# burn-research/OpenMEASURE

Measured on AMD Instinct MI355X. Metric: SPR fit+reconstruct throughput (GB/s snapshot matrix), higher is better.
Workload: dtype f64

## Files before the change

openmeasure_amd/csrc/common.hpp:

```cpp
#pragma once
#include <hip/hip_runtime.h>
#include <stdint.h>
#include <stdio.h>

#include "spr_hip.h"

typedef double f64x4 __attribute__((ext_vector_type(4)));
typedef double f64x2 __attribute__((ext_vector_type(2)));

void spr_set_error(const char *fmt, ...);

#define SPR_REQUIRE(cond, code, ...)      \
  do {                                    \
    if (!(cond)) {                        \
      spr_set_error(__VA_ARGS__);         \
      return (code);                      \
    }                                     \
  } while (0)

#define SPR_HIP_TRY(expr)                                                          \
  do {                                                                             \
    hipError_t e__ = (expr);                                                       \
    if (e__ != hipSuccess) {                                                       \
      spr_set_error("%s failed: %s (%s:%d)", #expr, hipGetErrorString(e__),       \
                    __FILE__, __LINE__);                                           \
      return SPR_E_HIP;                                                            \
    }                                                                              \
  } while (0)

#define SPR_LAUNCH_CHECK()                                                         \
  do {                                                                             \
    hipError_t e__ = hipGetLastError();                                            \
    if (e__ != hipSuccess) {                                                       \
      spr_set_error("kernel launch failed: %s (%s:%d)", hipGetErrorString(e__),   \
                    __FILE__, __LINE__);                                           \
      return SPR_E_HIP;                                                            \
    }                                                                              \
  } while (0)

int spr_cached_cus();

struct SegPlan {
  int64_t row0, n_rows, n_points;
  int32_t n_features;
  int32_t total_wg;
  int32_t chunk_rows;
};

__host__ __device__ inline void seg_range(const SegPlan &p, int f, int64_t &lo, int64_t &hi) {
  int64_t glo = (int64_t)f * p.n_points, ghi = glo + p.n_points;
  if (glo < p.row0) glo = p.row0;
  if (ghi > p.row0 + p.n_rows) ghi = p.row0 + p.n_rows;
  if (ghi < glo) ghi = glo;
  lo = glo - p.row0;
  hi = ghi - p.row0;
}

__host__ __device__ inline int seg_wgs(const SegPlan &p, int64_t rows) {
  if (rows <= 0) return 0;
  int64_t w = rows * (int64_t)p.total_wg / p.n_rows;
  int64_t chunks = (rows + p.chunk_rows - 1) / p.chunk_rows;
  if (w > chunks) w = chunks;
  if (w < 1) w = 1;
  return (int)w;
}

__host__ __device__ inline int seg_first_feature(const SegPlan &p) { return (int)(p.row0 / p.n_points); }
__host__ __device__ inline int seg_last_feature(const SegPlan &p) {
  int64_t f = (p.row0 + p.n_rows - 1) / p.n_points;
  if (f > p.n_features - 1) f = p.n_features - 1;
  return (int)f;
}

// ... 65 lines not shown
```

openmeasure_amd/csrc/project_ws.hip:

```cpp
#include <type_traits>

#include "rowtile.hpp"

namespace {

#ifndef WS_ABLATE
#define WS_ABLATE 0
#endif
constexpr int WS_WAVES = 8;
constexpr int WS_ROWS = 16 * WS_WAVES;

template <int RT> struct WsLds { static constexpr int NC = 16 * RT, LDW = NC; static_assert(RT % 2 == 0, "column tiles come in pairs"); };

template <typename TX> struct WsPiece;
template <> struct WsPiece<double> { f64x2 a, b; };
template <> struct WsPiece<float> { float x, y, z, w; };

template <int VEC, typename TX>
__device__ inline WsPiece<TX> ws_load(const TX *__restrict__ rp, int col0, int m) {
  WsPiece<TX> p;
  if constexpr (std::is_same<TX, double>::value) {
    if (VEC) {
      p.a = *reinterpret_cast<const f64x2 *>(rp + col0);
      p.b = *reinterpret_cast<const f64x2 *>(rp + col0 + 2);
    } else {
      p.a.x = rp[col0 < m ? col0 : 0];         p.a.y = rp[col0 + 1 < m ? col0 + 1 : 0];
      p.b.x = rp[col0 + 2 < m ? col0 + 2 : 0]; p.b.y = rp[col0 + 3 < m ? col0 + 3 : 0];
    }
  } else {
    if (VEC) {
      const float4 v = *reinterpret_cast<const float4 *>(rp + col0);
      p.x = v.x; p.y = v.y; p.z = v.z; p.w = v.w;
    } else {
      p.x = rp[col0 < m ? col0 : 0];         p.y = rp[col0 + 1 < m ? col0 + 1 : 0];
      p.z = rp[col0 + 2 < m ? col0 + 2 : 0]; p.w = rp[col0 + 3 < m ? col0 + 3 : 0];
    }
  }
  return p;
}

template <typename TX>
__device__ inline double ws_elem(const WsPiece<TX> &p, int t) {
  if constexpr (std::is_same<TX, double>::value) return t == 0 ? p.a.x : t == 1 ? p.a.y : t == 2 ? p.b.x : p.b.y;
  else return (double)(t == 0 ? p.x : t == 1 ? p.y : t == 2 ? p.z : p.w);
}

template <int MT, int RT, int VEC, typename TX, typename TU, bool NRM>
__global__ __launch_bounds__(WS_WAVES * 64) void project_ws_kernel(
    const TX *__restrict__ X, int64_t ldx, int m, int center_i, SegPlan plan, const double *__restrict__ inv_scale,
    const double *__restrict__ rowmean, const double *__restrict__ W, int r, TU *__restrict__ Ur, int64_t ldu,
    double *__restrict__ nrm2) {
  constexpr int K = 16 * MT, NJ = MT;
  constexpr int NC = WsLds<RT>::NC, LDW = WsLds<RT>::LDW;
  __shared__ double Wl[K * LDW];

  int f, wl, wpf, base;
  int64_t lo, hi;
  if (!seg_locate(plan, blockIdx.x, f, wl, wpf, base, lo, hi)) return;

  const int lane = threadIdx.x & 63;
  const int wave = __builtin_amdgcn_readfirstlane(threadIdx.x >> 6);
  const int li = lane & 15, kk = lane >> 4;
  const double isc = inv_scale[f];

  for (int e = threadIdx.x; e < K * NC; e += WS_WAVES * 64) {
    const int k = e / NC, c = e - k * NC;
    Wl[k * LDW + (c >> 5) * 32 + (c & 15) * 2 + ((c >> 4) & 1)] = (k < m && c < r) ? W[(int64_t)k * r + c] * isc : 0.0;
  }
  __syncthreads();
  double wbar[RT];
#pragma unroll
  for (int ct = 0; ct < RT; ++ct) {
    double sacc = 0.0;
    if (center_i != 0) {
      for (int k = kk; k < K; k += 4) sacc += Wl[k * LDW + (ct >> 1) * 32 + li * 2 + (ct & 1)];
      sacc += __shfl_xor(sacc, 16, 64);
      sacc += __shfl_xor(sacc, 32, 64);
    }
    wbar[ct] = sacc;
  }

  const int64_t nchunks = (hi - lo + WS_ROWS - 1) / WS_ROWS;
  int64_t c = wl;
  if (c >= nchunks) return;
  const double *wb = Wl + (4 * kk) * LDW + 2 * li;
  const double *wb_hi = wb + 128 * LDW;

  auto row_ptr = [&](int64_t cc) {
    int64_t row = lo + cc * WS_ROWS + 16 * wave + li;
    row = row < hi ? row : hi - 1;
    return X + row * ldx;
  };
  WsPiece<TX> areg[NJ];
  {
    const TX *rp = row_ptr(c);
#pragma unroll
    for (int j = 0; j < NJ; ++j) areg[j] = ws_load<VEC, TX>(rp, 16 * j + 4 * kk, m);
  }
  while (c < nchunks) {
    const int64_t cn = c + wpf;
    const TX *rpn = row_ptr(cn < nchunks ? cn : c);
    const int64_t blk0 = lo + c * WS_ROWS + 16 * wave;
    double mu[4];
#pragma unroll
    for (int i = 0; i < 4; ++i) {
      const int64_t rr = blk0 + kk + 4 * i;
      const double v = rowmean[rr < hi ? rr : hi - 1];
      mu[i] = center_i != 0 ? v : 0.0;
    }
    f64x4 acc[RT];
#pragma unroll
    for (int ct = 0; ct < RT; ++ct) acc[ct] = (f64x4){0.0, 0.0, 0.0, 0.0};
    f64x2 bcur[RT / 2], bnxt[RT / 2];
#pragma unroll
    for (int p = 0; p < RT / 2; ++p) bcur[p] = *reinterpret_cast<const f64x2 *>(wb + 32 * p);
#pragma unroll
    for (int j = 0; j < NJ; ++j) {
// ... 22 lines not shown
        for (int p = 0; p < RT / 2; ++p) bcur[p] = bnxt[p];
      }
    }
    {
      const bool full = (blk0 + 16 <= hi) && (r == NC);
      TU *up = Ur + (blk0 + kk) * ldu + li;
      double q[4] = {0.0, 0.0, 0.0, 0.0};
#pragma unroll
      for (int ct = 0; ct < RT; ++ct) {
        const double s[4] = {acc[ct].x - mu[0] * wbar[ct], acc[ct].y - mu[1] * wbar[ct],
                             acc[ct].z - mu[2] * wbar[ct], acc[ct].w - mu[3] * wbar[ct]};
        if (NRM) {
#pragma unroll
          for (int i = 0; i < 4; ++i) { const double v = (double)(TU)s[i]; q[i] = fma(v, v, q[i]); }
        }
        if (full) {
#pragma unroll
          for (int i = 0; i < 4; ++i) up[4 * i * ldu + 16 * ct] = (TU)s[i];
        } else if (16 * ct + li < r) {
#pragma unroll
          for (int i = 0; i < 4; ++i)
            if (blk0 + kk + 4 * i < hi) up[4 * i * ldu + 16 * ct] = (TU)s[i];
        }
      }
      if (NRM) {
#pragma unroll
        for (int i = 0; i < 4; ++i) {
          const double t = group_sum_t<16>(q[i]);
          if (li == i && blk0 + kk + 4 * i < hi) nrm2[blk0 + kk + 4 * i] = t;
        }
      }
    }
    c = cn;
  }
}

template <int MT, int RT, typename TX, typename TU>
int ws_launch(const TX *X, int64_t n_rows, int32_t m, int64_t ldx, int64_t row0, int64_t n_points, int32_t n_features,
              int center, const double *inv_scale, const double *rowmean, const double *W, int32_t r, TU *Ur,
              int64_t ldu, int accumulate, double *nrm2, hipStream_t st) {
  const int cus = spr_cached_cus();
  SegPlan plan;
  plan.row0 = row0; plan.n_rows = n_rows; plan.n_points = n_points; plan.n_features = n_features;
  static const int narrow_per_cu = [] { const char *e = getenv("SPR_WS_WG_PER_CU"); const int v = e ? atoi(e) : 2; return v >= 1 && v <= 4 ? v : 2; }();
  plan.total_wg = (cus > 0 ? cus : 256) * (MT <= 4 ? narrow_per_cu : 1);
  plan.chunk_rows = WS_ROWS;
  const int grid = seg_total_wgs(plan);
  const bool vec = (m == 16 * MT) && ((sizeof(TX) * ldx) % 16 == 0) && ((reinterpret_cast<uintptr_t>(X) & 15) == 0);
  if (!vec) return SPR_E_UNSUPPORTED;
  if (nrm2)
    hipLaunchKernelGGL((project_ws_kernel<MT, RT, 1, TX, TU, true>), dim3(grid), dim3(WS_WAVES * 64), 0, st, X, ldx, (int)m,
                       center, plan, inv_scale, rowmean, W, (int)r, Ur, ldu, nrm2);
  else
    hipLaunchKernelGGL((project_ws_kernel<MT, RT, 1, TX, TU, false>), dim3(grid), dim3(WS_WAVES * 64), 0, st, X, ldx, (int)m,
                       center, plan, inv_scale, rowmean, W, (int)r, Ur, ldu, nrm2);
  SPR_LAUNCH_CHECK();
  return SPR_OK;
}

}

#include "project_ws.hpp"

template <typename TX, typename TU>
int spr_project_ws(const TX *d_X, int64_t n_rows, int32_t m, int64_t ldx, int64_t row0, int64_t n_points,
                   int32_t n_features, int32_t center, const double *d_inv_scale, const double *d_rowmean,
                   const double *d_W, int32_t r, TU *d_Ur, int64_t ldu, int32_t accumulate, double *d_rownorm2,
                   hipStream_t st) {
  if (accumulate) return SPR_E_UNSUPPORTED;
  const int mt = spr_round_mt(m);
  const int need = (r + 15) / 16;
  const int rt = need <= 2 ? 2 : need <= 4 ? 4 : 0;
#define WS(MTV, RTV)                                                                                             \
  if (mt == MTV && rt == RTV)                                                                                    \
    return ws_launch<MTV, RTV, TX, TU>(d_X, n_rows, m, ldx, row0, n_points, n_features, center, d_inv_scale,   \
                                        d_rowmean, d_W, r, d_Ur, ldu, accumulate, d_rownorm2, st)
#ifdef PROJ_WS_LAB
  WS(16, 4);
#else
  WS(4, 2); WS(4, 4); WS(8, 2); WS(8, 4); WS(12, 2); WS(12, 4); WS(16, 2); WS(16, 4);
#endif
#undef WS
  return SPR_E_UNSUPPORTED;
}

template int spr_project_ws<double, double>(const double *, int64_t, int32_t, int64_t, int64_t, int64_t, int32_t, int32_t,
                                            const double *, const double *, const double *, int32_t, double *, int64_t,
                                            int32_t, double *, hipStream_t);
// ... 9 lines not shown
```

openmeasure_amd/csrc/runtime.hip:

```cpp
#include <stdarg.h>
#include <stdlib.h>
#include <string.h>

#include "common.hpp"

namespace {
thread_local char g_err[512] = "";
}

void spr_set_error(const char *fmt, ...) {
  va_list ap;
  va_start(ap, fmt);
  vsnprintf(g_err, sizeof(g_err), fmt, ap);
  va_end(ap);
}

int spr_cached_cus() {
  static int cus = 0;
  if (cus) return cus;
  int dev = 0;
  hipDeviceProp_t prop;
  if (hipGetDevice(&dev) != hipSuccess || hipGetDeviceProperties(&prop, dev) != hipSuccess) return 0;
  cus = prop.multiProcessorCount;
  if (const char *e = getenv("SPR_RESERVE_CUS")) {
    const int k = atoi(e);
    if (k > 0 && k < cus) cus -= k;
  }
  return cus;
}

extern "C" int spr_abi_version(void) { return SPR_ABI_VERSION; }

extern "C" const char *spr_last_error(void) { return g_err; }

extern "C" int spr_device_cus(int *out_cus) {
  SPR_REQUIRE(out_cus != nullptr, SPR_E_INVALID, "spr_device_cus: NULL output");
  const int c = spr_cached_cus();
  SPR_REQUIRE(c > 0, SPR_E_HIP, "spr_device_cus: no HIP device");
  *out_cus = c;
  return SPR_OK;
}

namespace {
__global__ __launch_bounds__(256) void upload_kernel(const uint64_t *__restrict__ src, uint64_t *__restrict__ dst,
                                                     int64_t n_words) {
  for (int64_t i = (int64_t)blockIdx.x * 256 + threadIdx.x; i < n_words; i += (int64_t)gridDim.x * 256)
    dst[i] = __builtin_nontemporal_load(src + i);
// ... 42 lines not shown
```

openmeasure_amd/csrc/stats_gram.hip:

```cpp
#include <stdlib.h>

#include <type_traits>

#include "rowtile.hpp"

#ifndef GRAM_UNIT_PAIRING
#define GRAM_UNIT_PAIRING 1
#endif
#ifndef GRAM_ABLATE
#define GRAM_ABLATE 0
#endif
#if GRAM_ABLATE == 1
#define GRAM_MFMA(a, b, c) ({ asm volatile("" ::"v"(a), "v"(b)); (c); })
#else
#define GRAM_MFMA(a, b, c) __builtin_amdgcn_mfma_f64_16x16x4f64((a), (b), (c), 0, 0, 0)
#endif

namespace {

template <int MT>
struct GramShape {
  static constexpr int MPAD = 16 * MT;
  static constexpr int MP = MPAD + ((MT % 2 == 0) ? 16 : 0);
  static constexpr int T = MT * (MT + 1) / 2;
  static constexpr int NU = (MT + 1) / 2;
};

template <int MT> struct GramCfg;
template <> struct GramCfg<1>  { static constexpr int NW = 8,  R = 64, KS = 8; static constexpr bool DBUF = true; static constexpr int LPRMAX = 16; };
template <> struct GramCfg<2>  { static constexpr int NW = 8,  R = 32, KS = 8; static constexpr bool DBUF = true; static constexpr int LPRMAX = 16; };
template <> struct GramCfg<3>  { static constexpr int NW = 8,  R = 64, KS = 4; static constexpr bool DBUF = true; static constexpr int LPRMAX = 16; };
#ifndef GRAM4_R
#define GRAM4_R 64
#define GRAM4_LPR 8
#endif
template <> struct GramCfg<4>  { static constexpr int NW = 8,  R = GRAM4_R, KS = 4; static constexpr bool DBUF = true; static constexpr int LPRMAX = GRAM4_LPR; };
// ... 146 lines not shown
    }
  }
  if (KSO == KS || ks == 0) {
    double *sp = slab + ((int64_t)blockIdx.x * KSO + (KSO == KS ? ks : 0)) * T * 256 + lane;
#pragma unroll
    for (int j = 0; j < NA; ++j) {
      double *tp = sp + (int64_t)tri_index(MT, RA, RA + j) * 256;
      tp[0] = accA[j].x; tp[64] = accA[j].y; tp[128] = accA[j].z; tp[192] = accA[j].w;
    }
#pragma unroll
    for (int j = 0; j < NB; ++j) {
      double *tp = sp + (int64_t)tri_index(MT, RB, RB + j) * 256;
      tp[0] = accB[j].x; tp[64] = accB[j].y; tp[128] = accB[j].z; tp[192] = accB[j].w;
    }
  }
  if ((lane % RT::LPR) == 0) {
    double *q = stat_part + ((int64_t)blockIdx.x * RT::ROWS_PER_IT + wave * RT::RPW + lane / RT::LPR) * 3;
    q[0] = st.cnt; q[1] = st.mean(); q[2] = st.m2();
  }
}

__device__ inline void chan_merge(double &n, double &mu, double &m2, double nb, double mb, double sb) {
  if (nb > 0.0) {
    const double tot = n + nb, d = mb - mu;
    mu += d * nb / tot;
    m2 += sb + d * d * n * nb / tot;
    n = tot;
  }
}

template <int MT, int U, typename TX, bool EXT, bool SUMS>
__device__ inline void gram_wave_own(const TX *__restrict__ X, int64_t ldx, int64_t lo, int64_t hi, int wl, int wpf, int ks,
                                     int wave, int lane, double *__restrict__ lds0, double *__restrict__ lds1,
                                     double *__restrict__ rowmean, double *__restrict__ slab, double *__restrict__ rowsum) {
  using S = GramShape<MT>;
  using C = GramCfg<MT>;
  constexpr int R = C::R, KS = C::KS, NW = C::NW, MP = S::MP, T = S::T;
  constexpr int KROWS = R / KS, KSTEPS = KROWS / 4;
  constexpr int RA = U, RB = MT - 1 - U;
  constexpr int NA = MT - RA;
  constexpr int NB = (RB != RA) ? MT - RB : 0;
  using RT = RowTile<MT, R, MP, NW, C::LPRMAX, TX>;

  f64x4 accA[NA];
  f64x4 accB[NB > 0 ? NB : 1];
#pragma unroll
  for (int j = 0; j < NA; ++j) accA[j] = (f64x4){0.0, 0.0, 0.0, 0.0};
#pragma unroll
  for (int j = 0; j < NB; ++j) accB[j] = (f64x4){0.0, 0.0, 0.0, 0.0};

  RT tile;
  const int64_t nchunks = (hi - lo + R - 1) / R;
  const int64_t lane_off = (int64_t)(wave * RT::RPW + lane / RT::LPR) * ldx;
  auto base_of = [&](int64_t row0) { return X + row0 * ldx; };
  int64_t c = wl;
  int64_t crow0 = lo + c * R;
#pragma unroll
  for (int it = 0; it < RT::IT; ++it) tile.template load_pass_own<EXT>(it, base_of(crow0), ldx, lane_off, hi - crow0, wave, lane, rowmean, crow0);
  if (crow0 + R <= hi) {
#pragma unroll
    for (int it = 0; it < RT::IT; ++it) tile.template center_store_own<true, EXT, SUMS>(it, lds0, crow0, hi - crow0, wave, lane, rowmean, rowsum);
  } else {
#pragma unroll
    for (int it = 0; it < RT::IT; ++it) tile.template center_store_own<false, EXT, SUMS>(it, lds0, crow0, hi - crow0, wave, lane, rowmean, rowsum);
  }
  int64_t cn = c + wpf;
  int64_t nrow0 = (cn < nchunks) ? lo + cn * R : hi;
// ... 23 lines not shown
      double op[2][NA];
#pragma unroll
      for (int j = 0; j < NA; ++j) op[0][j] = p[16 * j];
#pragma unroll
      for (int k = 0; k < KSTEPS; ++k) {
        if (k + 1 < KSTEPS) {
#pragma unroll
          for (int j = 0; j < NA; ++j) op[(k + 1) & 1][j] = p[(k + 1) * 4 * MP + 16 * j];
        }
#pragma unroll
        for (int j = 0; j < NA; ++j) accA[j] = GRAM_MFMA(op[k & 1][0], op[k & 1][j], accA[j]);
#pragma unroll
        for (int j = 0; j < NB; ++j) accB[j] = GRAM_MFMA(op[k & 1][RB - RA], op[k & 1][RB - RA + j], accB[j]);
        if (nfull) stage(std::true_type{}, k); else stage(std::false_type{}, k);
      }
    } else {
#pragma unroll
      for (int k = 0; k < KSTEPS; ++k) {
        double op[NA];
#pragma unroll
        for (int j = 0; j < NA; ++j) op[j] = p[k * 4 * MP + 16 * j];
#pragma unroll
        for (int j = 0; j < NA; ++j) accA[j] = GRAM_MFMA(op[0], op[j], accA[j]);
#pragma unroll
        for (int j = 0; j < NB; ++j) accB[j] = GRAM_MFMA(op[RB - RA], op[RB - RA + j], accB[j]);
        if (nfull) stage(std::true_type{}, k); else stage(std::false_type{}, k);
      }
    }
    buf ^= 1;
    c = cn;
    cn = c2;
    nrow0 = n2row0;
  }
  double *sp = slab + ((int64_t)blockIdx.x * KS + ks) * T * 256 + lane;
#pragma unroll
  for (int j = 0; j < NA; ++j) {
    double *tp = sp + (int64_t)tri_index(MT, RA, RA + j) * 256;
    tp[0] = accA[j].x; tp[64] = accA[j].y; tp[128] = accA[j].z; tp[192] = accA[j].w;
  }
#pragma unroll
  for (int j = 0; j < NB; ++j) {
    double *tp = sp + (int64_t)tri_index(MT, RB, RB + j) * 256;
    tp[0] = accB[j].x; tp[64] = accB[j].y; tp[128] = accB[j].z; tp[192] = accB[j].w;
  }
}

template <int MT, typename TX, bool EXT, bool SUMS>
__global__ __launch_bounds__(GramCfg<MT>::NW * 64) void stats_gram_own_kernel(
    const TX *__restrict__ X, int64_t ldx, SegPlan plan, double *__restrict__ rowmean, double *__restrict__ slab,
    double *__restrict__ rowsum) {
  using S = GramShape<MT>;
  using C = GramCfg<MT>;
  constexpr int NU = S::NU;
  __shared__ double lds[2][C::R * S::MP];
  int f, wl, wpf, base;
  int64_t lo, hi;
  if (!seg_locate(plan, blockIdx.x, f, wl, wpf, base, lo, hi)) return;
  const int lane = threadIdx.x & 63;
  const int wave = __builtin_amdgcn_readfirstlane(threadIdx.x >> 6);
  const int ks = wave / NU;
  const int unit = (GRAM_UNIT_PAIRING && NU == 8 && C::KS == 1) ? ((wave < 4) ? wave : 11 - wave) : wave % NU;
#define GRAM_UNIT(UV)                                                                                          \
  case UV:                                                                                                     \
    if constexpr (UV < NU)                                                                                     \
      gram_wave_own<MT, UV, TX, EXT, SUMS>(X, ldx, lo, hi, wl, wpf, ks, wave, lane, lds[0], lds[1], rowmean, slab, rowsum); \
    break;
  switch (unit) {
    GRAM_UNIT(0) GRAM_UNIT(1) GRAM_UNIT(2) GRAM_UNIT(3) GRAM_UNIT(4) GRAM_UNIT(5) GRAM_UNIT(6) GRAM_UNIT(7)
    default: break;
  }
#undef GRAM_UNIT
}

constexpr int RS_THREADS = 1024;
__global__ __launch_bounds__(RS_THREADS) void gram_rowmean_stats_kernel(const double *__restrict__ rowmean, SegPlan plan,
                                                                        int slots_per_wg, double *__restrict__ stat_part) {
  __shared__ double sn[RS_THREADS / 64], smu[RS_THREADS / 64], sm2[RS_THREADS / 64];
  int f, wl, wpf, base;
  int64_t lo, hi;
  if (!seg_locate(plan, blockIdx.x, f, wl, wpf, base, lo, hi)) return;
  const int lane = threadIdx.x & 63, wave = threadIdx.x >> 6;
  RowStats st;
  st.init();
  const int64_t step = (int64_t)wpf * RS_THREADS;
  int64_t row = lo + (int64_t)wl * RS_THREADS + threadIdx.x;
  for (; row + 3 * step < hi; row += 4 * step) {
    const double a = rowmean[row], b = rowmean[row + step], c = rowmean[row + 2 * step], d = rowmean[row + 3 * step];
    st.push(a, true); st.push(b, true); st.push(c, true); st.push(d, true);
  }
  for (; row < hi; row += step) st.push(rowmean[row], true);
  double n = st.cnt, mu = st.mean(), m2 = st.m2();
  for (int o = 32; o > 0; o >>= 1) {
    const double on = __shfl_down(n, o, 64), om = __shfl_down(mu, o, 64), os = __shfl_down(m2, o, 64);
    chan_merge(n, mu, m2, on, om, os);
  }
  if (lane == 0) { sn[wave] = n; smu[wave] = mu; sm2[wave] = m2; }
  __syncthreads();
  double *q = stat_part + (int64_t)blockIdx.x * slots_per_wg * 3;
  if (threadIdx.x == 0) {
    n = 0.0; mu = 0.0; m2 = 0.0;
    for (int w = 0; w < RS_THREADS / 64; ++w) chan_merge(n, mu, m2, sn[w], smu[w], sm2[w]);
    q[0] = n; q[1] = mu; q[2] = m2;
  }
  for (int e = 3 + threadIdx.x; e < slots_per_wg * 3; e += RS_THREADS) q[e] = 0.0;
}

template <int MT, int VEC, typename TX>
__global__ __launch_bounds__(GramCfg<MT>::NW * 64) void stats_gram_kernel(
    const TX *__restrict__ X, int64_t ldx, int m, int center_i, SegPlan plan,
    double *__restrict__ rowmean, double *__restrict__ stat_part, double *__restrict__ slab, double *__restrict__ rowsum) {
  using S = GramShape<MT>;
  using C = GramCfg<MT>;
  constexpr int NU = S::NU;
  static_assert(NU * C::KS == C::NW, "waves = units x k slices");
  __shared__ double lds[2][C::R * S::MP];

  int f, wl, wpf, base;
  int64_t lo, hi;
  if (!seg_locate(plan, blockIdx.x, f, wl, wpf, base, lo, hi)) return;

  const int lane = threadIdx.x & 63;
  const int wave = __builtin_amdgcn_readfirstlane(threadIdx.x >> 6);
  const int unit = wave % NU, ks = wave / NU;
#define GRAM_UNIT(UV)                                                                                        \
  case UV:                                                                                                   \
    if constexpr (UV < NU)                                                                                   \
      gram_wave<MT, UV, VEC, TX>(X, ldx, m, center_i, lo, hi, wl, wpf, ks, wave, lane, lds[0],    \
                        lds[1], rowmean, stat_part, slab, rowsum);                                           \
    break;
  switch (unit) {
    GRAM_UNIT(0) GRAM_UNIT(1) GRAM_UNIT(2) GRAM_UNIT(3) GRAM_UNIT(4) GRAM_UNIT(5) GRAM_UNIT(6) GRAM_UNIT(7)
    default: break;
  }
#undef GRAM_UNIT
}

template <int MT>
__global__ __launch_bounds__(1024) void gram_finalize_kernel(
    const double *__restrict__ slab, const double *__restrict__ stat_part, int m, SegPlan plan,
    int slots_per_wg, double *__restrict__ gram, double *__restrict__ fstats, int ldg, int origin) {
  constexpr int T = GramShape<MT>::T;
  constexpr int KS = GramOut<MT>::KSO;
  __shared__ double red[4][256];
  const int f = blockIdx.y;
  const int tile = blockIdx.x;
  int base = 0, wpf = 0;
  {
    int acc = 0;
    const int f0 = seg_first_feature(plan), f1 = seg_last_feature(plan);
    for (int ff = f0; ff <= f1; ++ff) {
      int64_t lo, hi;
      seg_range(plan, ff, lo, hi);
      const int w = seg_wgs(plan, hi - lo);
      if (ff == f) { base = acc; wpf = w; }
      acc += w;
    }
  }
  int ti, tj;
  tile_coords<MT>(tile, ti, tj);
  const int e = threadIdx.x & 255, g = threadIdx.x >> 8;
  const int np = wpf * KS;
  const double *sp = slab + ((int64_t)base * KS * T + tile) * 256 + e;
  const int64_t stride = (int64_t)T * 256;
  double s0 = 0.0, s1 = 0.0, s2 = 0.0, s3 = 0.0;
  int p = g;
  for (; p + 12 < np; p += 16) {
    s0 += sp[p * stride];
    s1 += sp[(p + 4) * stride];
    s2 += sp[(p + 8) * stride];
    s3 += sp[(p + 12) * stride];
  }
  for (; p < np; p += 4) s0 += sp[p * stride];
  red[g][e] = (s0 + s1) + (s2 + s3);
  __syncthreads();
  if (g == 0) {
    const double sum = (red[0][e] + red[1][e]) + (red[2][e] + red[3][e]);
    const int l = e & 63, reg = e >> 6;
    const int gi = ti * 16 + (l >> 4) + 4 * reg, gj = tj * 16 + (l & 15);
    if (gi < m && gj < m) {
      double *G = gram + (int64_t)f * ldg * ldg + (int64_t)origin * ldg + origin;
// ... 22 lines not shown
    }
  }
}

template <int MT>
int occupancy_wgs() {
  static int cached = 0;
  if (cached) return cached;
  int per_cu = 0;
  if (hipOccupancyMaxActiveBlocksPerMultiprocessor(&per_cu, stats_gram_kernel<MT, 2, double>, GramCfg<MT>::NW * 64, 0) != hipSuccess ||
      per_cu < 1)
    per_cu = 1;
  if (per_cu > 4) per_cu = 4;
  const int cus = spr_cached_cus();
  cached = per_cu * (cus > 0 ? cus : 256);
  return cached;
}

template <int MT>
SegPlan make_plan(int64_t n_rows, int64_t row0, int64_t n_points, int32_t n_features) {
  SegPlan p;
  p.row0 = row0; p.n_rows = n_rows; p.n_points = n_points; p.n_features = n_features;
  p.total_wg = occupancy_wgs<MT>();
  p.chunk_rows = GramCfg<MT>::R;
  return p;
}

template <int MT>
size_t workspace_bytes(int32_t n_features) {
  using RT = RowTile<MT, GramCfg<MT>::R, GramShape<MT>::MP, GramCfg<MT>::NW, GramCfg<MT>::LPRMAX>;
  const int64_t max_grid = (int64_t)occupancy_wgs<MT>() + n_features;
  return (size_t)max_grid * GramCfg<MT>::KS * GramShape<MT>::T * 256 * sizeof(double) +
         (size_t)max_grid * RT::ROWS_PER_IT * 3 * sizeof(double);
}

template <int MT, typename TX>
int launch(const TX *X, int64_t n_rows, int32_t m, int64_t ldx, int64_t row0, int64_t n_points,
           int32_t n_features, int center, double *rowmean, void *ws, size_t ws_bytes, hipStream_t st,
           double *rowsum = nullptr) {
  SPR_REQUIRE(ws_bytes >= workspace_bytes<MT>(n_features), SPR_E_WORKSPACE,
              "spr_stats_gram_f64: workspace %zu < %zu", ws_bytes, workspace_bytes<MT>(n_features));
  SPR_REQUIRE(!rowsum || center == 2, SPR_E_INVALID, "spr_stats_gram: row sums are an output of centre mode 2 only");
  SegPlan plan = make_plan<MT>(n_rows, row0, n_points, n_features);
  const int grid = seg_total_wgs(plan);
  const int64_t max_grid = (int64_t)occupancy_wgs<MT>() + n_features;
  SPR_REQUIRE(grid >= 1 && grid <= max_grid, SPR_E_INVALID, "spr_stats_gram_f64: bad grid %d", grid);
  double *slab = static_cast<double *>(ws);
  double *stat_part = slab + (size_t)max_grid * GramCfg<MT>::KS * GramShape<MT>::T * 256;
  const int vec_ok = (m % 2 == 0) && (ldx % 2 == 0) && ((reinterpret_cast<uintptr_t>(X) & (2 * sizeof(TX) - 1)) == 0);
  const int lm = vec_ok ? ((m == 16 * MT) ? 2 : 1) : 0;
#define SG_LAUNCH(LM)                                                                                         \
  hipLaunchKernelGGL((stats_gram_kernel<MT, LM, TX>), dim3(grid), dim3(GramCfg<MT>::NW * 64), 0, st, X, ldx, (int)m, \
                     center, plan, rowmean, stat_part, slab, rowsum)
  using RTL = RowTile<MT, GramCfg<MT>::R, GramShape<MT>::MP, GramCfg<MT>::NW, GramCfg<MT>::LPRMAX, TX>;
  static const bool own_on = [] { const char *e = getenv("SPR_GRAM_OWN"); return !(e && e[0] == '0'); }();
  if (MT >= 8 && lm == 2 && (center == 1 || center == 2) && own_on && (sizeof(TX) * ldx) % 16 == 0 &&
      (reinterpret_cast<uintptr_t>(X) & 15) == 0) {
    if constexpr (MT >= 8) {
      if (center == 1)
        hipLaunchKernelGGL((stats_gram_own_kernel<MT, TX, false, false>), dim3(grid), dim3(GramCfg<MT>::NW * 64), 0, st, X, ldx,
                           plan, rowmean, slab, rowsum);
      else if (!rowsum)
        hipLaunchKernelGGL((stats_gram_own_kernel<MT, TX, true, false>), dim3(grid), dim3(GramCfg<MT>::NW * 64), 0, st, X, ldx,
                           plan, rowmean, slab, rowsum);
      else
        hipLaunchKernelGGL((stats_gram_own_kernel<MT, TX, true, true>), dim3(grid), dim3(GramCfg<MT>::NW * 64), 0, st, X, ldx,
                           plan, rowmean, slab, rowsum);
      SPR_LAUNCH_CHECK();
      hipLaunchKernelGGL(gram_rowmean_stats_kernel, dim3(grid), dim3(RS_THREADS), 0, st, rowmean, plan, (int)RTL::ROWS_PER_IT,
                         stat_part);
      SPR_LAUNCH_CHECK();
      return SPR_OK;
    }
  }
  if (lm == 2) SG_LAUNCH(2);
  else if (lm == 1) SG_LAUNCH(1);
  else SG_LAUNCH(0);
#undef SG_LAUNCH
  SPR_LAUNCH_CHECK();
  return SPR_OK;
}

template <int MT>
int launch_finalize(int64_t n_rows, int32_t m, int64_t row0, int64_t n_points, int32_t n_features,
                    double *fstats, double *gram, int ldg, int origin, const void *ws, size_t ws_bytes,
                    hipStream_t st) {
  using RT = RowTile<MT, GramCfg<MT>::R, GramShape<MT>::MP, GramCfg<MT>::NW, GramCfg<MT>::LPRMAX>;
  SPR_REQUIRE(ws_bytes >= workspace_bytes<MT>(n_features), SPR_E_WORKSPACE,
              "spr_stats_gram_finalize_f64: workspace %zu < %zu", ws_bytes, workspace_bytes<MT>(n_features));
  SegPlan plan = make_plan<MT>(n_rows, row0, n_points, n_features);
  const int64_t max_grid = (int64_t)occupancy_wgs<MT>() + n_features;
  const double *slab = static_cast<const double *>(ws);
  const double *stat_part = slab + (size_t)max_grid * GramCfg<MT>::KS * GramShape<MT>::T * 256;
  hipLaunchKernelGGL(gram_finalize_kernel<MT>, dim3(GramShape<MT>::T, n_features), dim3(1024), 0, st, slab,
                     stat_part, (int)m, plan, (int)RT::ROWS_PER_IT, gram, fstats, ldg, origin);
  SPR_LAUNCH_CHECK();
  return SPR_OK;
}

int check_args(const char *who, const void *X, int64_t n_rows, int32_t m, int64_t ldx, int64_t row0,
               int64_t n_points, int32_t n_features) {
  SPR_REQUIRE(X != nullptr, SPR_E_INVALID, "%s: X is NULL", who);
  SPR_REQUIRE(n_rows > 0 && m > 0 && ldx >= m, SPR_E_INVALID, "%s: bad shape n_rows=%lld m=%d ldx=%lld", who,
              (long long)n_rows, m, (long long)ldx);
  SPR_REQUIRE(n_points > 0 && n_features > 0 && row0 >= 0, SPR_E_INVALID, "%s: bad feature layout", who);
  SPR_REQUIRE(row0 + n_rows <= n_points * (int64_t)n_features, SPR_E_INVALID,
              "%s: rows [%lld,%lld) exceed n_points*n_features=%lld", who, (long long)row0,
              (long long)(row0 + n_rows), (long long)(n_points * (int64_t)n_features));
  SPR_REQUIRE(m <= SPR_MAX_M, SPR_E_UNSUPPORTED, "%s: m=%d > %d not built", who, m, SPR_MAX_M);
  return SPR_OK;
}

}

#define SPR_DISPATCH_MT(mt, CALL)            \
  switch (mt) {                              \
    case 1: CALL(1); break;                  \
    case 2: CALL(2); break;                  \
    case 3: CALL(3); break;                  \
    case 4: CALL(4); break;                  \
    case 6: CALL(6); break;                  \
    case 8: CALL(8); break;                  \
    case 12: CALL(12); break;                \
    case 16: CALL(16); break;                \
    default: break;                          \
  }

extern "C" size_t spr_stats_gram_workspace(int32_t m, int32_t n_features) {
// ... 86 lines not shown
```

Before: 1175.

## Add piece-based work partitioning so workgroups span multiple features in gram/projection

```diff
diff --git a/openmeasure_amd/csrc/common.hpp b/openmeasure_amd/csrc/common.hpp
--- a/openmeasure_amd/csrc/common.hpp
+++ b/openmeasure_amd/csrc/common.hpp
@@ -39,6 +39,7 @@
   } while (0)
 
 int spr_cached_cus();
+int spr_piece_plan_mask();
 
 struct SegPlan {
   int64_t row0, n_rows, n_points;
diff --git a/openmeasure_amd/csrc/piece_plan.hpp b/openmeasure_amd/csrc/piece_plan.hpp
--- /dev/null
+++ b/openmeasure_amd/csrc/piece_plan.hpp
@@ -0,0 +1,167 @@
+#pragma once
+#include <stdint.h>
+
+#if defined(__HIPCC__)
+#define PP_HD __host__ __device__ inline
+#else
+#define PP_HD inline
+#endif
+
+struct PiecePlan {
+  int64_t row0, n_rows, n_points;
+  int32_t n_features;
+  int32_t total_wg;
+  int32_t chunk_rows;
+};
+
+struct Piece {
+  int32_t f;
+  int32_t slot;
+  int64_t lo, hi;
+  int32_t wl, wpf;
+};
+
+PP_HD int64_t pp_ceil_div(int64_t a, int64_t b) { return (a + b - 1) / b; }
+
+PP_HD int pp_first_feature(const PiecePlan &p) { return (int)(p.row0 / p.n_points); }
+PP_HD int pp_last_feature(const PiecePlan &p) {
+  int64_t f = (p.row0 + p.n_rows - 1) / p.n_points;
+  if (f > p.n_features - 1) f = p.n_features - 1;
+  return (int)f;
+}
+
+PP_HD void pp_range(const PiecePlan &p, int f, int64_t &lo, int64_t &hi) {
+  int64_t glo = (int64_t)f * p.n_points, ghi = glo + p.n_points;
+  if (glo < p.row0) glo = p.row0;
+  if (ghi > p.row0 + p.n_rows) ghi = p.row0 + p.n_rows;
+  if (ghi < glo) ghi = glo;
+  lo = glo - p.row0;
+  hi = ghi - p.row0;
+}
+
+PP_HD int64_t pp_panels(const PiecePlan &p, int f) {
+  int64_t lo, hi;
+  pp_range(p, f, lo, hi);
+  return pp_ceil_div(hi - lo, p.chunk_rows);
+}
+
+PP_HD int64_t pp_total_panels(const PiecePlan &p) {
+  int64_t tot = 0;
+  for (int f = pp_first_feature(p); f <= pp_last_feature(p); ++f) tot += pp_panels(p, f);
+  return tot;
+}
+
+PP_HD bool pp_dense(const PiecePlan &p) { return p.n_rows >= (int64_t)p.total_wg * p.chunk_rows; }
+
+PP_HD bool pp_usable(const PiecePlan &p) {
+  if (p.n_rows <= 0 || p.total_wg <= 0 || p.chunk_rows <= 0 || p.n_points <= 0) return false;
+  return pp_dense(p) || pp_total_panels(p) <= 2 * (int64_t)p.total_wg;
+}
+
+PP_HD int pp_grid(const PiecePlan &p) {
+  if (pp_dense(p)) return p.total_wg;
+  const int64_t P = pp_total_panels(p);
+  return (int)(P < p.total_wg ? P : p.total_wg);
+}
+
+PP_HD int64_t pp_cut(const PiecePlan &p, int64_t b) { return b * p.n_rows / p.total_wg; }
+
+PP_HD int pp_feature_of(const PiecePlan &p, int64_t row) {
+  int64_t f = (p.row0 + row) / p.n_points;
+  if (f > p.n_features - 1) f = p.n_features - 1;
+  return (int)f;
+}
+
+PP_HD int64_t pp_snap(const PiecePlan &p, int64_t x) {
+  if (x >= p.n_rows) return p.n_rows;
+  int64_t lo, hi;
+  pp_range(p, pp_feature_of(p, x), lo, hi);
+  const int64_t s = lo + pp_ceil_div(x - lo, p.chunk_rows) * p.chunk_rows;
+  return s < hi ? s : hi;
+}
+
+PP_HD int pp_wg_of_row(const PiecePlan &p, int64_t x) {
+  int64_t b = pp_ceil_div((x + 1) * p.total_wg, p.n_rows) - 1;
+  if (b > p.total_wg - 1) b = p.total_wg - 1;
+  return (int)b;
+}
+
+PP_HD void pp_sparse_panel(const PiecePlan &p, int64_t g, Piece &pc) {
+  int64_t acc = 0;
+  const int f1 = pp_last_feature(p);
+  for (int f = pp_first_feature(p); f <= f1; ++f) {
+    int64_t lo, hi;
+    pp_range(p, f, lo, hi);
+    const int64_t c = pp_ceil_div(hi - lo, p.chunk_rows);
+    if (g < acc + c || f == f1) {
+      pc.f = f;
+      pc.slot = (int32_t)g;
+      pc.lo = lo + (g - acc) * p.chunk_rows;
+      pc.hi = pc.lo + p.chunk_rows < hi ? pc.lo + p.chunk_rows : hi;
+      if (pc.hi < pc.lo) pc.hi = pc.lo;
+      pc.wl = 0;
+      pc.wpf = 1;
+      return;
+    }
+    acc += c;
+  }
+}
+
+PP_HD int pp_num_pieces(const PiecePlan &p, int b) {
+  if (pp_dense(p)) return pp_feature_of(p, pp_cut(p, b + 1) - 1) - pp_feature_of(p, pp_cut(p, b)) + 1;
+  const int64_t P = pp_total_panels(p);
+  return (b < P ? 1 : 0) + ((int64_t)b + p.total_wg < P ? 1 : 0);
+}
+
+PP_HD void pp_piece(const PiecePlan &p, int b, int k, bool strided, Piece &pc) {
+  if (!pp_dense(p)) {
+    pp_sparse_panel(p, k == 0 ? (int64_t)b : (int64_t)b + p.total_wg, pc);
+    return;
+  }
+  const int f_lo = pp_feature_of(p, pp_cut(p, b)), f_hi = pp_feature_of(p, pp_cut(p, b + 1) - 1);
+  const int f = f_lo + k;
+  int64_t flo, fhi;
+  pp_range(p, f, flo, fhi);
+  pc.f = f;
+  pc.slot = b + (f - pp_first_feature(p));
+  if (f_lo == f_hi && strided) {
+    const int64_t b0 = pp_ceil_div(flo * p.total_wg, p.n_rows);
+    int64_t b1 = pp_ceil_div((fhi + 1) * p.total_wg, p.n_rows) - 1;
+    if (b1 > p.total_wg) b1 = p.total_wg;
+    pc.lo = pp_snap(p, pp_cut(p, b0));
+    pc.hi = pp_snap(p, pp_cut(p, b1));
+    pc.wl = (int32_t)(b - b0);
+    pc.wpf = (int32_t)(b1 - b0);
+    return;
+  }
+  const int64_t S = pp_snap(p, pp_cut(p, b)), E = pp_snap(p, pp_cut(p, b + 1));
+  pc.lo = S > flo ? S : flo;
+  pc.hi = E < fhi ? E : fhi;
+  if (pc.hi < pc.lo) pc.hi = pc.lo;
+  pc.wl = 0;
+  pc.wpf = 1;
+}
+
+PP_HD void pp_feature_slots(const PiecePlan &p, int f, int &slot0, int &n) {
+  slot0 = 0;
+  n = 0;
+  if (f < pp_first_feature(p) || f > pp_last_feature(p)) return;
+  int64_t lo, hi;
+  pp_range(p, f, lo, hi);
+  if (hi <= lo) return;
+  if (pp_dense(p)) {
+    const int bA = pp_wg_of_row(p, lo), bB = pp_wg_of_row(p, hi - 1);
+    slot0 = bA + (f - pp_first_feature(p));
+    n = bB - bA + 1;
+    return;
+  }
+  int64_t acc = 0;
+  for (int ff = pp_first_feature(p); ff < f; ++ff) acc += pp_panels(p, ff);
+  slot0 = (int)acc;
+  n = (int)pp_panels(p, f);
+}
+
+PP_HD int pp_slot_bound(const PiecePlan &p) {
+  if (pp_dense(p)) return p.total_wg + (pp_last_feature(p) - pp_first_feature(p));
+  return (int)pp_total_panels(p);
+}
diff --git a/openmeasure_amd/csrc/project_ws.hip b/openmeasure_amd/csrc/project_ws.hip
--- a/openmeasure_amd/csrc/project_ws.hip
+++ b/openmeasure_amd/csrc/project_ws.hip
@@ -1,5 +1,6 @@
 #include <type_traits>
 
+#include "piece_plan.hpp"
 #include "rowtile.hpp"
 
 namespace {
@@ -49,40 +50,56 @@
 __global__ __launch_bounds__(WS_WAVES * 64) void project_ws_kernel(
     const TX *__restrict__ X, int64_t ldx, int m, int center_i, SegPlan plan, const double *__restrict__ inv_scale,
     const double *__restrict__ rowmean, const double *__restrict__ W, int r, TU *__restrict__ Ur, int64_t ldu,
-    double *__restrict__ nrm2) {
+    double *__restrict__ nrm2, int pieces) {
   constexpr int K = 16 * MT, NJ = MT;
   constexpr int NC = WsLds<RT>::NC, LDW = WsLds<RT>::LDW;
   __shared__ double Wl[K * LDW];
 
-  int f, wl, wpf, base;
-  int64_t lo, hi;
-  if (!seg_locate(plan, blockIdx.x, f, wl, wpf, base, lo, hi)) return;
+  const PiecePlan pp = {plan.row0, plan.n_rows, plan.n_points, plan.n_features, plan.total_wg, plan.chunk_rows};
+  const int npieces = pieces ? pp_num_pieces(pp, blockIdx.x) : 1;
 
   const int lane = threadIdx.x & 63;
   const int wave = __builtin_amdgcn_readfirstlane(threadIdx.x >> 6);
   const int li = lane & 15, kk = lane >> 4;
-  const double isc = inv_scale[f];
-
-  for (int e = threadIdx.x; e < K * NC; e += WS_WAVES * 64) {
-    const int k = e / NC, c = e - k * NC;
-    Wl[k * LDW + (c >> 5) * 32 + (c & 15) * 2 + ((c >> 4) & 1)] = (k < m && c < r) ? W[(int64_t)k * r + c] * isc : 0.0;
-  }
-  __syncthreads();
+  int fcur = -1;
   double wbar[RT];
-#pragma unroll
-  for (int ct = 0; ct < RT; ++ct) {
-    double sacc = 0.0;
-    if (center_i != 0) {
-      for (int k = kk; k < K; k += 4) sacc += Wl[k * LDW + (ct >> 1) * 32 + li * 2 + (ct & 1)];
-      sacc += __shfl_xor(sacc, 16, 64);
-      sacc += __shfl_xor(sacc, 32, 64);
-    }
-    wbar[ct] = sacc;
+
+  for (int pk = 0; pk < npieces; ++pk) {
+  int f, wl, wpf;
+  int64_t lo, hi;
+  if (pieces) {
+    Piece pc;
+    pp_piece(pp, blockIdx.x, pk, true, pc);
+    f = pc.f; lo = pc.lo; hi = pc.hi; wl = pc.wl; wpf = pc.wpf;
+    if (lo + (int64_t)wl * WS_ROWS >= hi) continue;
+  } else {
+    int base;
+    if (!seg_locate(plan, blockIdx.x, f, wl, wpf, base, lo, hi)) return;
+  }
+  if (f != fcur) {
+    if (fcur >= 0) __syncthreads();
+    fcur = f;
+    const double isc = inv_scale[f];
+    for (int e = threadIdx.x; e < K * NC; e += WS_WAVES * 64) {
+      const int k = e / NC, c = e - k * NC;
+      Wl[k * LDW + (c >> 5) * 32 + (c & 15) * 2 + ((c >> 4) & 1)] = (k < m && c < r) ? W[(int64_t)k * r + c] * isc : 0.0;
+    }
+    __syncthreads();
+#pragma unroll
+    for (int ct = 0; ct < RT; ++ct) {
+      double sacc = 0.0;
+      if (center_i != 0) {
+        for (int k = kk; k < K; k += 4) sacc += Wl[k * LDW + (ct >> 1) * 32 + li * 2 + (ct & 1)];
+        sacc += __shfl_xor(sacc, 16, 64);
+        sacc += __shfl_xor(sacc, 32, 64);
+      }
+      wbar[ct] = sacc;
+    }
   }
 
   const int64_t nchunks = (hi - lo + WS_ROWS - 1) / WS_ROWS;
   int64_t c = wl;
-  if (c >= nchunks) return;
+  if (c >= nchunks) continue;
   const double *wb = Wl + (4 * kk) * LDW + 2 * li;
   const double *wb_hi = wb + 128 * LDW;
 
@@ -171,6 +188,7 @@
       }
     }
     c = cn;
+  }
   }
 }
 
@@ -184,15 +202,17 @@
   static const int narrow_per_cu = [] { const char *e = getenv("SPR_WS_WG_PER_CU"); const int v = e ? atoi(e) : 2; return v >= 1 && v <= 4 ? v : 2; }();
   plan.total_wg = (cus > 0 ? cus : 256) * (MT <= 4 ? narrow_per_cu : 1);
   plan.chunk_rows = WS_ROWS;
-  const int grid = seg_total_wgs(plan);
   const bool vec = (m == 16 * MT) && ((sizeof(TX) * ldx) % 16 == 0) && ((reinterpret_cast<uintptr_t>(X) & 15) == 0);
   if (!vec) return SPR_E_UNSUPPORTED;
+  const PiecePlan pp = {row0, n_rows, n_points, n_features, plan.total_wg, plan.chunk_rows};
+  const int pieces = (MT >= 8 && std::is_same<TX, double>::value && (spr_piece_plan_mask() & 2) && pp_usable(pp)) ? 1 : 0;
+  const int grid = pieces ? pp_grid(pp) : seg_total_wgs(plan);
   if (nrm2)
     hipLaunchKernelGGL((project_ws_kernel<MT, RT, 1, TX, TU, true>), dim3(grid), dim3(WS_WAVES * 64), 0, st, X, ldx, (int)m,
-                       center, plan, inv_scale, rowmean, W, (int)r, Ur, ldu, nrm2);
+                       center, plan, inv_scale, rowmean, W, (int)r, Ur, ldu, nrm2, pieces);
   else
     hipLaunchKernelGGL((project_ws_kernel<MT, RT, 1, TX, TU, false>), dim3(grid), dim3(WS_WAVES * 64), 0, st, X, ldx, (int)m,
-                       center, plan, inv_scale, rowmean, W, (int)r, Ur, ldu, nrm2);
+                       center, plan, inv_scale, rowmean, W, (int)r, Ur, ldu, nrm2, pieces);
   SPR_LAUNCH_CHECK();
   return SPR_OK;
 }
diff --git a/openmeasure_amd/csrc/runtime.hip b/openmeasure_amd/csrc/runtime.hip
--- a/openmeasure_amd/csrc/runtime.hip
+++ b/openmeasure_amd/csrc/runtime.hip
@@ -13,6 +13,11 @@
   va_start(ap, fmt);
   vsnprintf(g_err, sizeof(g_err), fmt, ap);
   va_end(ap);
+}
+
+int spr_piece_plan_mask() {
+  static const int mask = [] { const char *e = getenv("SPR_PIECE_PLAN"); return e ? (atoi(e) & 3) : 1; }();
+  return mask;
 }
 
 int spr_cached_cus() {
diff --git a/openmeasure_amd/csrc/stats_gram.hip b/openmeasure_amd/csrc/stats_gram.hip
--- a/openmeasure_amd/csrc/stats_gram.hip
+++ b/openmeasure_amd/csrc/stats_gram.hip
@@ -2,6 +2,7 @@
 
 #include <type_traits>
 
+#include "piece_plan.hpp"
 #include "rowtile.hpp"
 
 #ifndef GRAM_UNIT_PAIRING
@@ -214,7 +215,8 @@
 template <int MT, int U, typename TX, bool EXT, bool SUMS>
 __device__ inline void gram_wave_own(const TX *__restrict__ X, int64_t ldx, int64_t lo, int64_t hi, int wl, int wpf, int ks,
                                      int wave, int lane, double *__restrict__ lds0, double *__restrict__ lds1,
-                                     double *__restrict__ rowmean, double *__restrict__ slab, double *__restrict__ rowsum) {
+                                     double *__restrict__ rowmean, double *__restrict__ slab, double *__restrict__ rowsum,
+                                     int slot) {
   using S = GramShape<MT>;
   using C = GramCfg<MT>;
   constexpr int R = C::R, KS = C::KS, NW = C::NW, MP = S::MP, T = S::T;
@@ -304,7 +306,7 @@
     cn = c2;
     nrow0 = n2row0;
   }
-  double *sp = slab + ((int64_t)blockIdx.x * KS + ks) * T * 256 + lane;
+  double *sp = slab + ((int64_t)slot * KS + ks) * T * 256 + lane;
 #pragma unroll
   for (int j = 0; j < NA; ++j) {
     double *tp = sp + (int64_t)tri_index(MT, RA, RA + j) * 256;
@@ -320,14 +322,13 @@
 template <int MT, typename TX, bool EXT, bool SUMS>
 __global__ __launch_bounds__(GramCfg<MT>::NW * 64) void stats_gram_own_kernel(
     const TX *__restrict__ X, int64_t ldx, SegPlan plan, double *__restrict__ rowmean, double *__restrict__ slab,
-    double *__restrict__ rowsum) {
+    double *__restrict__ rowsum, int pieces) {
   using S = GramShape<MT>;
   using C = GramCfg<MT>;
   constexpr int NU = S::NU;
   __shared__ double lds[2][C::R * S::MP];
-  int f, wl, wpf, base;
-  int64_t lo, hi;
-  if (!seg_locate(plan, blockIdx.x, f, wl, wpf, base, lo, hi)) return;
+  const PiecePlan pp = {plan.row0, plan.n_rows, plan.n_points, plan.n_features, plan.total_wg, plan.chunk_rows};
+  const int npieces = pieces ? pp_num_pieces(pp, blockIdx.x) : 1;
   const int lane = threadIdx.x & 63;
   const int wave = __builtin_amdgcn_readfirstlane(threadIdx.x >> 6);
   const int ks = wave / NU;
@@ -335,23 +336,56 @@
 #define GRAM_UNIT(UV)                                                                                          \
   case UV:                                                                                                     \
     if constexpr (UV < NU)                                                                                     \
-      gram_wave_own<MT, UV, TX, EXT, SUMS>(X, ldx, lo, hi, wl, wpf, ks, wave, lane, lds[0], lds[1], rowmean, slab, rowsum); \
+      gram_wave_own<MT, UV, TX, EXT, SUMS>(X, ldx, lo, hi, wl, wpf, ks, wave, lane, lds[0], lds[1], rowmean, slab, rowsum, slot); \
     break;
-  switch (unit) {
-    GRAM_UNIT(0) GRAM_UNIT(1) GRAM_UNIT(2) GRAM_UNIT(3) GRAM_UNIT(4) GRAM_UNIT(5) GRAM_UNIT(6) GRAM_UNIT(7)
-    default: break;
+  for (int k = 0; k < npieces; ++k) {
+    int wl, wpf, slot;
+    int64_t lo, hi;
+    if (pieces) {
+      Piece pc;
+      pp_piece(pp, blockIdx.x, k, true, pc);
+      lo = pc.lo; hi = pc.hi; wl = pc.wl; wpf = pc.wpf; slot = pc.slot;
+      if (lo + (int64_t)wl * C::R >= hi) {
+        double *z = slab + (int64_t)slot * C::KS * S::T * 256;
+        for (int e = threadIdx.x; e < C::KS * S::T * 256; e += C::NW * 64) z[e] = 0.0;
+        continue;
+      }
+      if (k > 0) __syncthreads();
+    } else {
+      int f, base;
+      if (!seg_locate(plan, blockIdx.x, f, wl, wpf, base, lo, hi)) return;
+      slot = blockIdx.x;
+    }
+    switch (unit) {
+      GRAM_UNIT(0) GRAM_UNIT(1) GRAM_UNIT(2) GRAM_UNIT(3) GRAM_UNIT(4) GRAM_UNIT(5) GRAM_UNIT(6) GRAM_UNIT(7)
+      default: break;
+    }
   }
 #undef GRAM_UNIT
 }
 
 constexpr int RS_THREADS = 1024;
 __global__ __launch_bounds__(RS_THREADS) void gram_rowmean_stats_kernel(const double *__restrict__ rowmean, SegPlan plan,
-                                                                        int slots_per_wg, double *__restrict__ stat_part) {
+                                                                        int slots_per_wg, double *__restrict__ stat_part,
+                                                                        int pieces, int64_t *__restrict__ layout) {
   __shared__ double sn[RS_THREADS / 64], smu[RS_THREADS / 64], sm2[RS_THREADS / 64];
-  int f, wl, wpf, base;
+  if (blockIdx.x == 0 && threadIdx.x == 0) *layout = pieces;
+  const PiecePlan pp = {plan.row0, plan.n_rows, plan.n_points, plan.n_features, plan.total_wg, plan.chunk_rows};
+  const int npieces = pieces ? pp_num_pieces(pp, blockIdx.x) : 1;
+  const int lane = threadIdx.x & 63, wave = threadIdx.x >> 6;
+  for (int k = 0; k < npieces; ++k) {
+  int wl, wpf, slot;
   int64_t lo, hi;
-  if (!seg_locate(plan, blockIdx.x, f, wl, wpf, base, lo, hi)) return;
-  const int lane = threadIdx.x & 63, wave = threadIdx.x >> 6;
+  if (pieces) {
+    Piece pc;
+    pp_piece(pp, blockIdx.x, k, false, pc);
+    lo = pc.lo; hi = pc.hi; wl = pc.wl; wpf = pc.wpf; slot = pc.slot;
+    if (k > 0) __syncthreads();
+  } else {
+    int f, base;
+    if (!seg_locate(plan, blockIdx.x, f, wl, wpf, base, lo, hi)) return;
+    slot = blockIdx.x;
+  }
   RowStats st;
   st.init();
   const int64_t step = (int64_t)wpf * RS_THREADS;
@@ -368,24 +402,27 @@
   }
   if (lane == 0) { sn[wave] = n; smu[wave] = mu; sm2[wave] = m2; }
   __syncthreads();
-  double *q = stat_part + (int64_t)blockIdx.x * slots_per_wg * 3;
+  double *q = stat_part + (int64_t)slot * slots_per_wg * 3;
   if (threadIdx.x == 0) {
     n = 0.0; mu = 0.0; m2 = 0.0;
     for (int w = 0; w < RS_THREADS / 64; ++w) chan_merge(n, mu, m2, sn[w], smu[w], sm2[w]);
     q[0] = n; q[1] = mu; q[2] = m2;
   }
   for (int e = 3 + threadIdx.x; e < slots_per_wg * 3; e += RS_THREADS) q[e] = 0.0;
+  }
 }
 
 template <int MT, int VEC, typename TX>
 __global__ __launch_bounds__(GramCfg<MT>::NW * 64) void stats_gram_kernel(
     const TX *__restrict__ X, int64_t ldx, int m, int center_i, SegPlan plan,
-    double *__restrict__ rowmean, double *__restrict__ stat_part, double *__restrict__ slab, double *__restrict__ rowsum) {
+    double *__restrict__ rowmean, double *__restrict__ stat_part, double *__restrict__ slab, double *__restrict__ rowsum,
+    int64_t *__restrict__ layout) {
   using S = GramShape<MT>;
   using C = GramCfg<MT>;
   constexpr int NU = S::NU;
   static_assert(NU * C::KS == C::NW, "waves = units x k slices");
   __shared__ double lds[2][C::R * S::MP];
+  if (blockIdx.x == 0 && threadIdx.x == 0) *layout = 0;
 
   int f, wl, wpf, base;
   int64_t lo, hi;
@@ -410,14 +447,18 @@
 template <int MT>
 __global__ __launch_bounds__(1024) void gram_finalize_kernel(
     const double *__restrict__ slab, const double *__restrict__ stat_part, int m, SegPlan plan,
-    int slots_per_wg, double *__restrict__ gram, double *__restrict__ fstats, int ldg, int origin) {
+    int slots_per_wg, double *__restrict__ gram, double *__restrict__ fstats, int ldg, int origin,
+    const int64_t *__restrict__ layout) {
   constexpr int T = GramShape<MT>::T;
   constexpr int KS = GramOut<MT>::KSO;
   __shared__ double red[4][256];
   const int f = blockIdx.y;
   const int tile = blockIdx.x;
   int base = 0, wpf = 0;
-  {
+  if (*layout != 0) {
+    const PiecePlan pp = {plan.row0, plan.n_rows, plan.n_points, plan.n_features, plan.total_wg, plan.chunk_rows};
+    pp_feature_slots(pp, f, base, wpf);
+  } else {
     int acc = 0;
     const int f0 = seg_first_feature(plan), f1 = seg_last_feature(plan);
     for (int ff = f0; ff <= f1; ++ff) {
@@ -506,6 +547,12 @@
   const int64_t max_grid = (int64_t)occupancy_wgs<MT>() + n_features;
   return (size_t)max_grid * GramCfg<MT>::KS * GramShape<MT>::T * 256 * sizeof(double) +
          (size_t)max_grid * RT::ROWS_PER_IT * 3 * sizeof(double);
+}
+
+template <int MT>
+int64_t *layout_word(double *stat_part, int64_t max_grid) {
+  using RT = RowTile<MT, GramCfg<MT>::R, GramShape<MT>::MP, GramCfg<MT>::NW, GramCfg<MT>::LPRMAX>;
+  return reinterpret_cast<int64_t *>(stat_part + (size_t)max_grid * RT::ROWS_PER_IT * 3 - 1);
 }
 
 template <int MT, typename TX>
@@ -525,24 +572,30 @@
   const int lm = vec_ok ? ((m == 16 * MT) ? 2 : 1) : 0;
 #define SG_LAUNCH(LM)                                                                                         \
   hipLaunchKernelGGL((stats_gram_kernel<MT, LM, TX>), dim3(grid), dim3(GramCfg<MT>::NW * 64), 0, st, X, ldx, (int)m, \
-                     center, plan, rowmean, stat_part, slab, rowsum)
+                     center, plan, rowmean, stat_part, slab, rowsum, layout)
   using RTL = RowTile<MT, GramCfg<MT>::R, GramShape<MT>::MP, GramCfg<MT>::NW, GramCfg<MT>::LPRMAX, TX>;
   static const bool own_on = [] { const char *e = getenv("SPR_GRAM_OWN"); return !(e && e[0] == '0'); }();
-  if (MT >= 8 && lm == 2 && (center == 1 || center == 2) && own_on && (sizeof(TX) * ldx) % 16 == 0 &&
-      (reinterpret_cast<uintptr_t>(X) & 15) == 0) {
+  const bool own = MT >= 8 && lm == 2 && (center == 1 || center == 2) && own_on && (sizeof(TX) * ldx) % 16 == 0 &&
+                   (reinterpret_cast<uintptr_t>(X) & 15) == 0;
+  const PiecePlan pp = {row0, n_rows, n_points, n_features, plan.total_wg, plan.chunk_rows};
+  const bool pieces = own && center == 1 && std::is_same<TX, double>::value && (spr_piece_plan_mask() & 1) && pp_usable(pp) &&
+                      pp_slot_bound(pp) < max_grid;
+  int64_t *layout = layout_word<MT>(stat_part, max_grid);
+  if (own) {
     if constexpr (MT >= 8) {
+      const int g = pieces ? pp_grid(pp) : grid;
       if (center == 1)
-        hipLaunchKernelGGL((stats_gram_own_kernel<MT, TX, false, false>), dim3(grid), dim3(GramCfg<MT>::NW * 64), 0, st, X, ldx,
-                           plan, rowmean, slab, rowsum);
+        hipLaunchKernelGGL((stats_gram_own_kernel<MT, TX, false, false>), dim3(g), dim3(GramCfg<MT>::NW * 64), 0, st, X, ldx,
+                           plan, rowmean, slab, rowsum, pieces ? 1 : 0);
       else if (!rowsum)
         hipLaunchKernelGGL((stats_gram_own_kernel<MT, TX, true, false>), dim3(grid), dim3(GramCfg<MT>::NW * 64), 0, st, X, ldx,
-                           plan, rowmean, slab, rowsum);
+                           plan, rowmean, slab, rowsum, 0);
       else
         hipLaunchKernelGGL((stats_gram_own_kernel<MT, TX, true, true>), dim3(grid), dim3(GramCfg<MT>::NW * 64), 0, st, X, ldx,
-                           plan, rowmean, slab, rowsum);
+                           plan, rowmean, slab, rowsum, 0);
       SPR_LAUNCH_CHECK();
-      hipLaunchKernelGGL(gram_rowmean_stats_kernel, dim3(grid), dim3(RS_THREADS), 0, st, rowmean, plan, (int)RTL::ROWS_PER_IT,
-                         stat_part);
+      hipLaunchKernelGGL(gram_rowmean_stats_kernel, dim3(g), dim3(RS_THREADS), 0, st, rowmean, plan, (int)RTL::ROWS_PER_IT,
+                         stat_part, pieces ? 1 : 0, layout);
       SPR_LAUNCH_CHECK();
       return SPR_OK;
     }
@@ -567,7 +620,8 @@
   const double *slab = static_cast<const double *>(ws);
   const double *stat_part = slab + (size_t)max_grid * GramCfg<MT>::KS * GramShape<MT>::T * 256;
   hipLaunchKernelGGL(gram_finalize_kernel<MT>, dim3(GramShape<MT>::T, n_features), dim3(1024), 0, st, slab,
-                     stat_part, (int)m, plan, (int)RT::ROWS_PER_IT, gram, fstats, ldg, origin);
+                     stat_part, (int)m, plan, (int)RT::ROWS_PER_IT, gram, fstats, ldg, origin,
+                     layout_word<MT>(const_cast<double *>(stat_part), max_grid));
   SPR_LAUNCH_CHECK();
   return SPR_OK;
 }
```

Result: no change. 1169 (-0.5%).
